# Nuralamsiddik16/Ultrafnd_git

Hardware: AMD Instinct MI355X
Metric: train-step samples/sec (FakeSV batch, seq128+224^2) (higher is better)
Workload: dtype bf16

## Files before the change

### ultrafnd_git_amd/csrc/attn_softmax.hpp

```cpp
#pragma once
#include "common.hpp"

#pragma clang fp contract(off)

__device__ __forceinline__ bf16x8 lds_frag(const char* tile, int row, int chunk) {
  return *reinterpret_cast<const bf16x8*>(tile + row * 128 + ((chunk ^ ((row >> 1) & 7)) << 4));
}

__device__ __forceinline__ bool masked_block_is_noop(const float* kb, int lane, const float (&m_run)[2]) {
  return __all(kb[lane] != 0.0f) && __all(m_run[0] > -1.0e30f && m_run[1] > -1.0e30f);
}

template <int KT, bool DROP = false, bool CAUSAL = false>
__device__ __forceinline__ float online_softmax_block(f32x4 (&s)[KT][2], const int qt, const float* kbias, const bool any_masked, const int g,
                                                      const float scale_log2e, float& m_run, float& l_run, bf16x8 (&pf)[KT / 2][2],
                                                      const f32x4* dm = nullptr, const int qk = 0, const float causal_neg = 0.0f) {
  float mx = -INFINITY, lsum = 0.0f, m_new, alpha;
  if (any_masked) {
#pragma unroll
    for (int kt = 0; kt < KT; ++kt) {
      const f32x4 kbv = *reinterpret_cast<const f32x4*>(kbias + kt * 16 + 4 * g);
#pragma unroll
      for (int r = 0; r < 4; ++r) {
        float v = (kbv[r] == 0.0f) ? s[kt][qt][r] * scale_log2e : kbv[r];
        if constexpr (CAUSAL) {
          if (kbv[r] == 0.0f && 16 * kt + r > qk) v = causal_neg;
        }
        s[kt][qt][r] = v;
        mx = fmaxf(mx, v);
      }
    }
    mx = fmaxf(mx, __shfl_xor(mx, 16, 64));
    mx = fmaxf(mx, __shfl_xor(mx, 32, 64));
    m_new = fmaxf(m_run, mx);
    alpha = fast_exp2(m_run - m_new);
#pragma unroll
    for (int kt = 0; kt < KT; ++kt)
#pragma unroll
      for (int r = 0; r < 4; ++r) {
        const float p = fast_exp2(s[kt][qt][r] - m_new);
        lsum += p;
        if constexpr (DROP) pf[kt >> 1][qt][(kt & 1) * 4 + r] = (__bf16)(p * dm[kt][r]);
        else pf[kt >> 1][qt][(kt & 1) * 4 + r] = (__bf16)p;
      }
  } else {
#pragma unroll
    for (int kt = 0; kt < KT; ++kt)
#pragma unroll
      for (int r = 0; r < 4; ++r) mx = fmaxf(mx, s[kt][qt][r]);
    mx = fmaxf(mx, __shfl_xor(mx, 16, 64));
    mx = fmaxf(mx, __shfl_xor(mx, 32, 64));
    m_new = fmaxf(m_run, mx * scale_log2e);
    alpha = fast_exp2(m_run - m_new);
    const float neg_m = -m_new;
#pragma unroll
    for (int kt = 0; kt < KT; ++kt)
#pragma unroll
      for (int r = 0; r < 4; ++r) {
        const float p = fast_exp2(__builtin_fmaf(s[kt][qt][r], scale_log2e, neg_m));
        lsum += p;
        if constexpr (DROP) pf[kt >> 1][qt][(kt & 1) * 4 + r] = (__bf16)(p * dm[kt][r]);
        else pf[kt >> 1][qt][(kt & 1) * 4 + r] = (__bf16)p;
      }
  }
  l_run = __builtin_fmaf(l_run, alpha, lsum);
  m_run = m_new;
  return alpha;
}

__device__ __forceinline__ void attn_init(f32x4 (&o)[4][2], float (&m_run)[2], float (&l_run)[2]) {
#pragma unroll
  for (int dt = 0; dt < 4; ++dt)
#pragma unroll
    for (int qt = 0; qt < 2; ++qt) o[dt][qt] = f32x4{0.f, 0.f, 0.f, 0.f};
#pragma unroll
  for (int qt = 0; qt < 2; ++qt) m_run[qt] = -INFINITY, l_run[qt] = 0.f;
}

template <class QRow>
__device__ __forceinline__ void attn_q_frags(const char* qimg, QRow q_row, int fr, int g, bf16x8 (&qf)[2][2]) {
#pragma unroll
  for (int qt = 0; qt < 2; ++qt) {
    const int row = q_row(qt * 16 + fr);
    qf[qt][0] = lds_frag(qimg, row, g);
    qf[qt][1] = lds_frag(qimg, row, g + 4);
  }
}

template <int KT, class KeyRow>
__device__ __forceinline__ void attn_scores(const char* kimg, KeyRow key_row, const bf16x8 (&qf)[2][2], int fr, int g, f32x4 (&s)[KT][2]) {
#pragma unroll
  for (int kt = 0; kt < KT; ++kt)
#pragma unroll
    for (int qt = 0; qt < 2; ++qt) s[kt][qt] = f32x4{0.f, 0.f, 0.f, 0.f};
#pragma unroll
  for (int kk = 0; kk < 2; ++kk)
#pragma unroll
    for (int kt = 0; kt < KT; ++kt) {
      const bf16x8 kf = lds_frag(kimg, key_row(kt * 16 + fr), g + 4 * kk);
#pragma unroll
      for (int qt = 0; qt < 2; ++qt) s[kt][qt] = __builtin_amdgcn_mfma_f32_16x16x32_bf16(kf, qf[qt][kk], s[kt][qt], 0, 0, 0);
    }
}

template <int KT, bool DROP = false, bool CAUSAL = false>
__device__ __forceinline__ void attn_softmax_rescale(f32x4 (&s)[KT][2], const int qt, const float* kbias, const bool any_masked, const int g,
                                                     const float scale_log2e, float (&m_run)[2], float (&l_run)[2], bf16x8 (&pf)[KT / 2][2],
                                                     f32x4 (&o)[4][2], const f32x4* dm = nullptr, const int qk = 0, const float causal_neg = 0.0f) {
  const float alpha = online_softmax_block<KT, DROP, CAUSAL>(s, qt, kbias, any_masked, g, scale_log2e, m_run[qt], l_run[qt], pf, dm, qk, causal_neg);
  if (!__all(alpha == 1.0f)) {
#pragma unroll
    for (int dt = 0; dt < 4; ++dt) o[dt][qt] *= alpha;
  }
}

template <int KT, class KeyRow>
__device__ __forceinline__ void attn_pv(const char* vimg, KeyRow key_row, const bf16x8 (&pf)[KT / 2][2], f32x4 (&o)[4][2], int fr, int g) {
#pragma unroll
  for (int ksd = 0; ksd < KT / 2; ++ksd) {
#pragma unroll
    for (int dt = 0; dt < 4; ++dt) {
      const int qq = fr >> 2, pp = fr & 3;
      const int k0 = 32 * ksd + 4 * g + qq;
      const int key0 = key_row(k0), key1 = key_row(k0 + 16);
      const int ch = 2 * dt + (pp >> 1);
      const int off0 = key0 * 128 + ((ch ^ (((key0 >> 1) & 3) << 1)) << 4) + 8 * (pp & 1);
      const int off1 = key1 * 128 + ((ch ^ (((key1 >> 1) & 3) << 1)) << 4) + 8 * (pp & 1);
      const s16x4 t0 = __builtin_amdgcn_ds_read_tr16_b64_v4i16((s16x4 __attribute__((address_space(3)))*)(vimg + off0));
      const s16x4 t1 = __builtin_amdgcn_ds_read_tr16_b64_v4i16((s16x4 __attribute__((address_space(3)))*)(vimg + off1));
      union { s16x4 s2[2]; bf16x8 v; } u;
      u.s2[0] = t0;
      u.s2[1] = t1;
#pragma unroll
      for (int qt = 0; qt < 2; ++qt) o[dt][qt] = __builtin_amdgcn_mfma_f32_16x16x32_bf16(u.v, pf[ksd][qt], o[dt][qt], 0, 0, 0);
    }
  }
}

__device__ __forceinline__ float attn_finish(const float l_run, float& l) {
  l = l_run;
  l += __shfl_xor(l, 16, 64);
  l += __shfl_xor(l, 32, 64);
  return 1.0f / l;
}
__device__ __forceinline__ float attn_finish(const float l_run) {
  float l;
  return attn_finish(l_run, l);
}

__device__ __forceinline__ void attn_store_ctx(__bf16* dst, const f32x4 (&o)[4][2], const int qt, const float inv) {
#pragma unroll
  for (int dt = 0; dt < 4; ++dt) {
    bf16x4 ov = {(__bf16)(o[dt][qt][0] * inv), (__bf16)(o[dt][qt][1] * inv), (__bf16)(o[dt][qt][2] * inv), (__bf16)(o[dt][qt][3] * inv)};
    *reinterpret_cast<bf16x4*>(dst + dt * 16) = ov;
  }
}
```

### ultrafnd_git_amd/csrc/common.hpp

```cpp
#pragma once
#include <hip/hip_runtime.h>
#include <stdint.h>
#include <stdio.h>

#include "../../include/ultrafnd_hip.h"

typedef float f32x16 __attribute__((ext_vector_type(16)));
typedef float f32x4 __attribute__((ext_vector_type(4)));
typedef float f32x2 __attribute__((ext_vector_type(2)));
typedef __bf16 bf16x8 __attribute__((ext_vector_type(8)));
typedef __bf16 bf16x4 __attribute__((ext_vector_type(4)));
typedef short s16x4 __attribute__((ext_vector_type(4)));

#define UFND_WAVE 64

void ufnd_set_error(const char* fmt, ...);
#define UFND_REQUIRE(cond, ...)                      \
  do {                                               \
    if (!(cond)) {                                   \
      ufnd_set_error(__VA_ARGS__);                   \
      return UFND_ERR_INVALID;                       \
    }                                                \
  } while (0)
#define UFND_CHECK_LAUNCH()                                              \
// ... 2 lines not shown
    if (e_ != hipSuccess) {                                              \
      ufnd_set_error("%s:%d launch failed: %s", __FILE__, __LINE__,      \
                     hipGetErrorString(e_));                             \
      return UFND_ERR_LAUNCH;                                            \
    }                                                                    \
  } while (0)

static inline bool ufnd_aligned(const void* p, size_t a) { return (reinterpret_cast<uintptr_t>(p) % a) == 0; }
static inline int ufnd_cdiv(int a, int b) { return (a + b - 1) / b; }

__device__ __forceinline__ float gelu_f(float x) {
  return 0.5f * x * (1.0f + erff(x * 0.70710678118654752440f));
}
__device__ __forceinline__ float gelu_grad_f(float x) {
  const float cdf = 0.5f * (1.0f + erff(x * 0.70710678118654752440f));
  const float pdf = 0.39894228040143267794f * __expf(-0.5f * x * x);
  return cdf + x * pdf;
}
__device__ __forceinline__ float sigmoid_f(float x) { return 1.0f / (1.0f + __expf(-x)); }
__device__ __forceinline__ int xcd_contiguous_id(int n, int total) {
  const int q = total >> 3, r = total & 7, xcd = n & 7, idx = n >> 3;
  return (xcd < r ? xcd * (q + 1) : r * (q + 1) + (xcd - r) * q) + idx;
}

__device__ __forceinline__ float fast_exp2(float x) { return __builtin_amdgcn_exp2f(x); }
__device__ __forceinline__ float quick_gelu_grad_f(float x) {
  const float s = 1.0f / (1.0f + __expf(-1.702f * x));
  return s * (1.0f + 1.702f * x * (1.0f - s));
}
__device__ __forceinline__ float sigmoid_fast_f(float x) {
#pragma clang fp contract(off)
  return __builtin_amdgcn_rcpf(__fadd_rn(1.0f, __expf(-x)));
}
__device__ __forceinline__ float quick_gelu_fast_f(float x) {
#pragma clang fp contract(off)
  return __fmul_rn(x, sigmoid_fast_f(__fmul_rn(1.702f, x)));
}
__device__ __forceinline__ float gelu_fast_f(float x) {
#pragma clang fp contract(off)
  const float z = __fmul_rn(fabsf(x), 0.70710678118654752440f);
  const float t = __builtin_amdgcn_rcpf(__fmaf_rn(0.3275911f, z, 1.0f));
  float p = __fmaf_rn(t, 1.061405429f, -1.453152027f);
  p = __fmaf_rn(t, p, 1.421413741f);
  p = __fmaf_rn(t, p, -0.284496736f);
  p = __fmaf_rn(t, p, 0.254829592f);
  const float poly = __fmul_rn(t, p);
  const float erf_abs = __fmaf_rn(-poly, __expf(__fmul_rn(-z, z)), 1.0f);
  const float h = __fmul_rn(0.5f, x);
  return __fmaf_rn(h, copysignf(erf_abs, x), h);
}

__device__ __forceinline__ f32x2 gelu_fast_f2(f32x2 x) {
#pragma clang fp contract(off)
  const f32x2 z = __builtin_elementwise_abs(x) * 0.70710678118654752440f;
  const f32x2 u = __builtin_elementwise_fma(f32x2{0.3275911f, 0.3275911f}, z, f32x2{1.0f, 1.0f});
  const f32x2 t = {__builtin_amdgcn_rcpf(u.x), __builtin_amdgcn_rcpf(u.y)};
  f32x2 p = __builtin_elementwise_fma(t, f32x2{1.061405429f, 1.061405429f}, f32x2{-1.453152027f, -1.453152027f});
  p = __builtin_elementwise_fma(t, p, f32x2{1.421413741f, 1.421413741f});
  p = __builtin_elementwise_fma(t, p, f32x2{-0.284496736f, -0.284496736f});
  p = __builtin_elementwise_fma(t, p, f32x2{0.254829592f, 0.254829592f});
  const f32x2 poly = t * p;
  const f32x2 zz = (-z) * z;
  const f32x2 e = {__expf(zz.x), __expf(zz.y)};
  const f32x2 erf_abs = __builtin_elementwise_fma(-poly, e, f32x2{1.0f, 1.0f});
  const f32x2 h = x * 0.5f;
  const f32x2 sg = {copysignf(erf_abs.x, x.x), copysignf(erf_abs.y, x.y)};
  return __builtin_elementwise_fma(h, sg, h);
}
__device__ __forceinline__ f32x2 quick_gelu_fast_f2(f32x2 x) {
#pragma clang fp contract(off)
  const f32x2 m = x * 1.702f;
  const f32x2 d = f32x2{__expf(-m.x), __expf(-m.y)} + 1.0f;
  const f32x2 r = {__builtin_amdgcn_rcpf(d.x), __builtin_amdgcn_rcpf(d.y)};
  return x * r;
}

__device__ __forceinline__ float quad_xor1(float v) {
  return __builtin_bit_cast(float, __builtin_amdgcn_update_dpp(0, __builtin_bit_cast(int, v), 0xB1, 0xF, 0xF, false));
}
__device__ __forceinline__ float quad_xor2(float v) {
  return __builtin_bit_cast(float, __builtin_amdgcn_update_dpp(0, __builtin_bit_cast(int, v), 0x4E, 0xF, 0xF, false));
}

#define UFND_DPP(v, old, ctrl, rmask) \
  __builtin_bit_cast(float, __builtin_amdgcn_update_dpp(__builtin_bit_cast(int, (float)(old)), __builtin_bit_cast(int, (float)(v)), ctrl, rmask, 0xF, false))
__device__ __forceinline__ float wave_sum(float v) {
  v += UFND_DPP(v, 0.0f, 0xB1, 0xF);
  v += UFND_DPP(v, 0.0f, 0x4E, 0xF);
  v += UFND_DPP(v, 0.0f, 0x141, 0xF);
  v += UFND_DPP(v, 0.0f, 0x140, 0xF);
  v += UFND_DPP(v, 0.0f, 0x142, 0xA);
  v += UFND_DPP(v, 0.0f, 0x143, 0xC);
  return __builtin_bit_cast(float, __builtin_amdgcn_readlane(__builtin_bit_cast(int, v), 63));
}
__device__ __forceinline__ float wave_max(float v) {
  v = fmaxf(v, UFND_DPP(v, v, 0xB1, 0xF));
  v = fmaxf(v, UFND_DPP(v, v, 0x4E, 0xF));
  v = fmaxf(v, UFND_DPP(v, v, 0x141, 0xF));
  v = fmaxf(v, UFND_DPP(v, v, 0x140, 0xF));
  v = fmaxf(v, UFND_DPP(v, v, 0x142, 0xA));
  v = fmaxf(v, UFND_DPP(v, v, 0x143, 0xC));
  return __builtin_bit_cast(float, __builtin_amdgcn_readlane(__builtin_bit_cast(int, v), 63));
}

__device__ __forceinline__ void philox_4x32(uint64_t seed, uint64_t step, uint32_t layer, uint32_t ctr, uint32_t (&out)[4]) {
  uint32_t k0 = (uint32_t)seed, k1 = (uint32_t)(seed >> 32);
  uint32_t c0 = ctr, c1 = layer, c2 = (uint32_t)step, c3 = (uint32_t)(step >> 32);
#pragma unroll
  for (int r = 0; r < 10; ++r) {
    const uint64_t p0 = (uint64_t)0xD2511F53u * c0;
    const uint64_t p1 = (uint64_t)0xCD9E8D57u * c2;
    const uint32_t n0 = (uint32_t)(p1 >> 32) ^ c1 ^ k0;
    const uint32_t n1 = (uint32_t)p1;
    const uint32_t n2 = (uint32_t)(p0 >> 32) ^ c3 ^ k1;
    const uint32_t n3 = (uint32_t)p0;
    c0 = n0; c1 = n1; c2 = n2; c3 = n3;
    k0 += 0x9E3779B9u; k1 += 0xBB67AE85u;
  }
  out[0] = c0; out[1] = c1; out[2] = c2; out[3] = c3;
}
__device__ __forceinline__ float dropout_keep(uint32_t r, float p) {
  const float u = (float)(r >> 8) * (1.0f / 16777216.0f);
  return (u >= p) ? 1.0f / (1.0f - p) : 0.0f;
}
__device__ __forceinline__ uint64_t dropout_step_key(const ufnd_step_state* st) { return st->step + ((uint64_t)st->micro << 40); }
__device__ __forceinline__ float dropout_mul(const ufnd_step_state* st, float p, uint32_t layer, uint32_t elem) {
  if (p <= 0.0f) return 1.0f;
  uint32_t w[4];
  philox_4x32(st->seed, dropout_step_key(st), layer, elem >> 2, w);
  const uint32_t k = elem & 3u;
  return dropout_keep(k == 0 ? w[0] : (k == 1 ? w[1] : (k == 2 ? w[2] : w[3])), p);
}
__device__ __forceinline__ void dropout_mul4(const ufnd_step_state* st, float p, uint32_t layer, uint32_t elem4, float (&m)[4]) {
  if (p <= 0.0f) { m[0] = m[1] = m[2] = m[3] = 1.0f; return; }
  uint32_t w[4];
  philox_4x32(st->seed, dropout_step_key(st), layer, elem4 >> 2, w);
#pragma unroll
  for (int q = 0; q < 4; ++q) m[q] = dropout_keep(w[q], p);
}
__device__ __forceinline__ void dropout_mul4_ctr(uint64_t seed, uint64_t step, float p, uint32_t layer, uint32_t ctr, float (&m)[4]) {
  uint32_t w[4];
  philox_4x32(seed, step, layer, ctr, w);
#pragma unroll
  for (int q = 0; q < 4; ++q) m[q] = dropout_keep(w[q], p);
}

static inline bool ufnd_attn_dropout_fits(int B, int L, int heads) {
  const long long lp = (L + 3) / 4 * 4;
  return (long long)B * heads * L * lp / 4 <= (1ll << 32);
}
constexpr uint32_t UFND_TAG_TEXT = 256;
constexpr uint32_t UFND_TAG_VISION = 4096;
```

### ultrafnd_git_amd/csrc/diag/gemm_diag.hip

```cpp
#define UFND_DIAG 1
#include "../gemm_bf16_kernel.hpp"
#include "../gemm_bf16_checks.hpp"

extern "C" int ufnd_diag_gemm_bf16_ex(const void* A, const void* W, const float* bias, const float* residual, void* out_bf16,
                                      float* out_f32, int M, int N, int K, int lda, int ldw, int ldr, int ldo, int ldf, int act,
                                      int tile_cfg, void* stream_) {
  UFND_REQUIRE(A && W && (out_bf16 || out_f32), "diag gemm: null operand");
  UFND_REQUIRE(M >= 1 && N >= 64 && K >= 64 && N % 64 == 0 && K % 64 == 0, "diag gemm: M=%d N=%d K=%d", M, N, K);
  GemmArgs a{(const __bf16*)A, (const __bf16*)W, bias, residual, (__bf16*)out_bf16, out_f32, M, N, K, lda, ldw, ldr, ldo, ldf, act, 0, 0, nullptr};
  int mode = 0, cfg = tile_cfg < 0 ? auto_cfg(M, N, K) : tile_cfg;
  if (cfg >= 200) { mode = 2; cfg -= 200; } else if (cfg >= 100) { mode = 1; cfg -= 100; }
  UFND_REQUIRE(cfg < kNumTiles, "diag gemm: unknown tile config %d", cfg);
  UFND_REQUIRE(N % kTiles[cfg].bn == 0, "diag gemm: tile config %d needs N %% %d == 0", cfg, kTiles[cfg].bn);
  int rc = launch_cfg(cfg, mode, a, (hipStream_t)stream_);
  if (rc != UFND_OK) return rc;
  UFND_CHECK_LAUNCH();
  return UFND_OK;
}

extern "C" int ufnd_diag_gemm_bf16_stamps(const void* A, const void* W, void* out_bf16, int M, int N, int K, int tile_cfg,
                                     unsigned long long* stamps, const ufnd_gemm_ln* ln, const float* bias, const float* residual,
                                     float* out_f32, void* stream_) {
  UFND_REQUIRE(A && W && out_bf16 && stamps, "gemm_bf16_stamps: null operand");
  UFND_REQUIRE(M >= 1 && N >= 64 && K >= 64 && N % 64 == 0 && K % 64 == 0, "gemm_bf16_stamps: M=%d N=%d K=%d", M, N, K);
  UFND_REQUIRE(tile_cfg >= 0 && tile_cfg < kNumTiles && N % kTiles[tile_cfg].bn == 0, "gemm_bf16_stamps: tile config %d", tile_cfg);
  GemmArgs a{(const __bf16*)A, (const __bf16*)W, bias, residual, (__bf16*)out_bf16, out_f32, M, N, K, K, K, N, N, N, 0, 0, 0, stamps};
  int abl = 3;
  if (ln) {
    UFND_REQUIRE(kTiles[tile_cfg].lnx, "gemm_bf16_stamps: tile %d has no LayerNorm-aware kernel", tile_cfg);
    a.a_stats = ln->a_stats; a.colsum = ln->colsum; a.r_stats = ln->r_stats; a.r_gamma = ln->r_gamma; a.r_beta = ln->r_beta;
    a.out_stats = ln->out_stats; a.a_parts = ln->a_parts; a.r_parts = ln->r_parts; a.a_eps = ln->a_eps; a.r_eps = ln->r_eps;
    a.inv_h = 1.0f / (float)ln->width;
    a.residual_b = (const __bf16*)ln->residual_bf16;
    a.ldrb = ln->ldrb;
    a.guard = ln->a_stats ? ln->guard : nullptr;
    if (ln->tile_cfg > 0) a.act = ln->tile_cfg;
    abl = 5;
  }
  int rc = launch_cfg(tile_cfg, abl, a, (hipStream_t)stream_);
  if (rc != UFND_OK) return rc;
  UFND_CHECK_LAUNCH();
  return UFND_OK;
}

extern "C" int ufnd_diag_qkv_attention_stamps(const void* X, const void* Wqkv, const float* bqkv, const int32_t* key_mask, void* ctx, int B,
                                              int heads, const ufnd_gemm_ln* ln, unsigned long long* stamps, void* stream_) {
  UFND_REQUIRE(X && Wqkv && ctx && stamps && heads % 2 == 0, "diag qkv_attention: bad argument");
  const int H = heads * 64;
  GemmArgs a{(const __bf16*)X, (const __bf16*)Wqkv, bqkv, nullptr, nullptr, nullptr, B * 128, 3 * H, H, H, H, 0, 0, 0, UFND_ACT_NONE, 0, 0, stamps};
  if (ln && ln->a_stats) {
    a.a_stats = ln->a_stats; a.colsum = ln->colsum; a.a_parts = ln->a_parts; a.a_eps = ln->a_eps;
    a.inv_h = 1.0f / (float)ln->width;
    a.guard = ln->guard;
  }
  a.att_mask = key_mask;
  a.att_ctx = (__bf16*)ctx;
  a.att_h = H;
  a.att_scale_log2e = 0.125f * 1.44269504088896340736f;
  a.m_tiles = B;
  a.n_tiles = heads / 2;
  a.xcd_cols = (a.n_tiles % 2 == 0 && a.m_tiles >= 4) ? 2 : 1;
  hipLaunchKernelGGL((gemm_bf16_kernel<128, 384, 2, 4, 3, 2, 16, 0, 1, 1, 1>), dim3(a.m_tiles * a.n_tiles), dim3(512), 0, (hipStream_t)stream_, a);
  UFND_CHECK_LAUNCH();
  return UFND_OK;
}

extern "C" int ufnd_diag_qkv_attention_tiles_stamps(const void* X, const void* Wqkv, const float* bqkv, const int32_t* tiles, const int32_t* ntiles,
                                                    void* ctx, int cap_tiles, int heads, const ufnd_gemm_ln* ln, unsigned long long* stamps,
                                                    void* stream_) {
  UFND_REQUIRE(X && Wqkv && ctx && stamps && tiles && ntiles && cap_tiles >= 1 && heads >= 1, "diag qkv_attention_tiles: bad argument");
  const int H = heads * 64;
  GemmArgs a{(const __bf16*)X, (const __bf16*)Wqkv, bqkv, nullptr, nullptr, nullptr, cap_tiles * 256, 3 * H, H, H, H, 0, 0, 0, UFND_ACT_NONE, 0, 0, stamps};
  if (ln && ln->a_stats) {
    a.a_stats = ln->a_stats; a.colsum = ln->colsum; a.a_parts = ln->a_parts; a.a_eps = ln->a_eps;
    a.inv_h = 1.0f / (float)ln->width;
    a.guard = ln->guard;
  }
  a.att_bins = tiles;
  a.att_nbins = ntiles;
  a.att_ctx = (__bf16*)ctx;
  a.att_h = H;
  a.att_scale_log2e = 0.125f * 1.44269504088896340736f;
  a.m_tiles = cap_tiles;
  a.n_tiles = heads;
  a.xcd_cols = 1;
  hipLaunchKernelGGL((gemm_bf16_kernel<256, 192, 4, 2, 3, 2, 16, 0, 1, 1, 2>), dim3(a.m_tiles * a.n_tiles), dim3(512), 0, (hipStream_t)stream_, a);
  UFND_CHECK_LAUNCH();
  return UFND_OK;
}

int ufnd_diag_pp_shape_ok(int M, int N, int K);
extern "C" int ufnd_diag_gemm_bf16_plan(int entry, const void* A, const void* W, const float* bias, const float* residual, const void* aux,
                                        const void* out_bf16, const float* out_f32, int M, int N, int K, int lda, int ldw, int ldr, int ldaux,
                                        int ldo, int ldf, int act, int tile_cfg, const ufnd_gemm_ln* ln, int* out) {
  UFND_REQUIRE(out, "gemm_bf16_plan: null result pointer");
  UFND_REQUIRE(entry >= -1 && entry <= 3, "gemm_bf16_plan: entry %d", entry);
  int cfg = tile_cfg, rc = UFND_OK, parts = 0;
  if (entry == -1) {
    UFND_REQUIRE(cfg >= 0 && cfg < kNumTiles, "gemm_bf16_plan: no tile %d", cfg);
    M = N = K = 0;
  } else if (entry == 3) {
    rc = gemm_bf16_dgrad_check_args(A, W, residual, aux, out_bf16, out_f32, M, N, K, lda, ldw, ldr, ldaux, ldo, ldf, act);
    if (rc != UFND_OK) return rc;
    cfg = auto_cfg(M, N, K);
    rc = gemm_bf16_dgrad_check_tile(cfg, N);
    if (rc != UFND_OK) return rc;
  } else {
    if (entry == 2) {
      rc = gemm_bf16_ln_check_args(A, W, bias, residual, out_bf16, out_f32, M, N, K, lda, ldw, ldr, ldo, ldf, act, ln);
      if (rc != UFND_OK) return rc;
      cfg = ln->tile_cfg;
    } else {
      rc = gemm_bf16_check_args(A, W, bias, residual, out_bf16, out_f32, M, N, K, lda, ldw, ldr, ldo, ldf, act);
      if (rc != UFND_OK) return rc;
      if (entry == 0) cfg = -1;
    }
    UFND_REQUIRE(cfg != UFND_GEMM_TILE_PERSISTENT && !(cfg < 0 && ufnd_diag_pp_shape_ok(M, N, K)),
                 "gemm_bf16_plan: the persistent form may take this call (its choice needs the device): not planned here");
    if (cfg < 0) cfg = auto_cfg(M, N, K);
    rc = entry == 2 ? gemm_bf16_ln_check_tile(cfg, M, N, K, ln) : gemm_bf16_check_tile(cfg, N);
    if (rc != UFND_OK) return rc;
    if (entry == 2 && ln->out_stats) parts = stat_parts_for(cfg, N);
  }
  const TileCfg& t = kTiles[cfg];
  const int m_tiles = entry < 0 ? 0 : ufnd_cdiv(M, t.bm), n_tiles = entry < 0 ? 0 : N / t.bn;
  out[0] = cfg;
  out[1] = m_tiles;
  out[2] = n_tiles;
  out[3] = entry < 0 ? 0 : xcd_cols_for(M, N, K, m_tiles, n_tiles);
  out[4] = parts;
  out[5] = t.bm; out[6] = t.bn; out[7] = t.sta; out[8] = t.stb; out[9] = t.lnx; out[10] = t.prod; out[11] = gemm_bwd_tile(cfg) ? 1 : 0;
  return UFND_OK;
}
```

### ultrafnd_git_amd/csrc/gemm_bf16_kernel.hpp

```cpp
#pragma once
#ifndef UFND_GEMM_OUT_NT
#define UFND_GEMM_OUT_NT 0
#endif

#include <type_traits>

#include "common.hpp"
#include "attn_softmax.hpp"

#pragma clang fp contract(off)

#ifndef UFND_GEMM_ILV
#define UFND_GEMM_ILV 1
#endif

namespace {

constexpr int BK = 64;

struct GemmArgs {
  const __bf16* A;
  const __bf16* W;
  const float* bias;
  const float* residual;
// ... 186 lines not shown
    }
    return tr < alen;
  };
  const int wave = __builtin_amdgcn_readfirstlane(threadIdx.x >> 6), lane = threadIdx.x & 63;
  const int wm = wave / WN, wn = wave % WN, fr = lane & (MI - 1), g = lane / MI;

  acc_t acc[MT][NT];
#pragma unroll
  for (int i = 0; i < MT; ++i)
#pragma unroll
    for (int j = 0; j < NT; ++j)
#pragma unroll
      for (int r = 0; r < AR; ++r) acc[i][j][r] = 0.f;

  int nk = a.K / BK, kbase = 0;
  if constexpr (BWD) {
    if (a.ksplit > 1) {
      const int per = (nk + a.ksplit - 1) / a.ksplit;
      kbase = kslice * per * BK;
      nk = nk - kslice * per < per ? nk - kslice * per : per;
    }
  }
  const int prow = lane >> 3, ppos = lane & 7;
  int arow_att[ATT ? PWA : 1];
  if constexpr (ATT) {
#pragma unroll
    for (int ii = 0; ii < PWA; ++ii) arow_att[ii] = tile_row(8 * (wave + NW * ii) + prow);
  }
  auto issueA = [&](int t, int kt) {
    char* buf = smem + (t % STA) * ASLOT;
    const int k0 = kbase + kt * BK;
#pragma unroll
    for (int ii = 0; ii < PWA; ++ii) {
      const int p = wave + NW * ii;
      const int r = 8 * p + prow;
      const int c = ppos ^ ((r >> 1) & 7);
      int gr = arow0 + r;
      gr = gr < mlive ? gr : mlive - 1;
      if constexpr (ATT) gr = arow_att[ii];
      dma16(a.A + (size_t)gr * a.lda + k0 + c * 8, buf + p * 1024);
    }
  };
  auto issueB = [&](int t, int kt) {
    char* buf = smem + STA * ASLOT + (t % STB) * BSLOT;
    const int k0 = kbase + kt * BK;
#pragma unroll
    for (int ii = 0; ii < PWB; ++ii) {
      int p = wave + NW * ii;
      if constexpr (BPIECES % NW != 0) p = p < BPIECES ? p : p - BPIECES;
      const int r = 8 * p + prow;
      const int c = ppos ^ ((r >> 1) & 7);
      int gr = n0 + r;
      gr = gr < a.N ? gr : a.N - 1;
      if constexpr (ONEH) gr = (r >> 6) * a.att_h + tn * 64 + (r & 63);
      else if constexpr (ATT) gr = (r >> 7) * a.att_h + tn * 128 + (r & 127);
      dma16(a.W + (size_t)gr * a.ldw + k0 + c * 8, buf + p * 1024);
    }
  };
  constexpr int TPR = NW * 64 / BM;
  static_assert(!LNX || TPR == 2 || TPR == 4, "threads per tile row");
  constexpr int GPT = 4 / (TPR < 4 ? TPR : 4);
  f32x4 sv[GPT][3];
  f32x2* st_lds = reinterpret_cast<f32x2*>(smem + STAT_OFF);
  const float* sp = nullptr;
  if constexpr (LNX) {
    sp = a.a_stats ? a.a_stats : a.r_stats;
    if (sp) {
      const int parts = a.a_stats ? a.a_parts : a.r_parts;
      int row = arow0 + (int)threadIdx.x / TPR;
      row = row < mlive ? row : mlive - 1;
      if constexpr (ATT) row = tile_row((int)threadIdx.x / TPR);
      const f32x4* base = reinterpret_cast<const f32x4*>(sp + (size_t)row * parts * 2);
      const int nq = parts >> 1, sub = threadIdx.x % TPR;
#pragma unroll
      for (int gi = 0; gi < GPT; ++gi)
#pragma unroll
        for (int u = 0; u < 3; ++u) {
          const int q = (sub + gi * TPR) + 4 * u;
          asm volatile("global_load_dwordx4 %0, %1, off" : "=v"(sv[gi][u]) : "v"(base + (q < nq ? q : 0)) : "memory");
        }
    }
  }
  float til_kb = 0.0f;
  if constexpr (TIL) {
    if (threadIdx.x < BM) til_kb = __int_as_float(til[UFND_TEXT_TILE_KBIAS + threadIdx.x]);
  }
  int att_mk = 1;
  if constexpr (ATT == 1 && !VIT) {
    if (slots) {
      const int j = (int)threadIdx.x >> 7, k = threadIdx.x & 127;
      const int mt = j == 0 ? smeta[0] : j == 1 ? smeta[1] : j == 2 ? smeta[2] : smeta[3];
      att_mk = mt >= 0 && k < (mt & 255);
      if (att_mk && a.att_mask) att_mk = a.att_mask[(size_t)(mt >> 10) * BM + k];
    } else if (a.att_mask && threadIdx.x < BM) {
      att_mk = a.att_mask[m0 + threadIdx.x];
    }
  }
#pragma unroll
  for (int s = 0; s < STA; ++s) {
    const int ks = s < nk ? s : nk - 1;
    if (s < STB && (LNX || s < nk)) issueB(s, ks);
    if (LNX || s < nk) issueA(s, ks);
  }

  if constexpr (LNX) {
    if (sp) {
      constexpr int NPRO = STA * PWA + STB * PWB;
      static_assert(NPRO <= 63, "vmcnt range");
      if constexpr (GPT == 1)
        asm volatile("s_waitcnt vmcnt(%3) ; STATRETIRE %0 %1 %2" : "+v"(sv[0][0]), "+v"(sv[0][1]), "+v"(sv[0][2]) : "n"(NPRO) : "memory");
      else
        asm volatile("s_waitcnt vmcnt(%6) ; STATRETIRE %0 %1 %2 %3 %4 %5" : "+v"(sv[0][0]), "+v"(sv[0][1]), "+v"(sv[0][2]), "+v"(sv[GPT - 1][0]),
                     "+v"(sv[GPT - 1][1]), "+v"(sv[GPT - 1][2]) : "n"(NPRO) : "memory");
      const int nq_ = (a.a_stats ? a.a_parts : a.r_parts) >> 1, sub_ = threadIdx.x % TPR;
      float gs[GPT], gq[GPT];
#pragma unroll
      for (int gi = 0; gi < GPT; ++gi) {
#pragma unroll
        for (int u = 0; u < 3; ++u) {
          if ((sub_ + gi * TPR) + 4 * u >= nq_) sv[gi][u] = f32x4{0.f, 0.f, 0.f, 0.f};
        }
        gs[gi] = sv[gi][0][0] + sv[gi][0][2];
        gq[gi] = sv[gi][0][1] + sv[gi][0][3];
#pragma unroll
        for (int u = 1; u < 3; ++u) { gs[gi] += sv[gi][u][0] + sv[gi][u][2]; gq[gi] += sv[gi][u][1] + sv[gi][u][3]; }
      }
      float sm, sq;
      if constexpr (TPR == 4) {
        sm = gs[0] + quad_xor1(gs[0]);
        sq = gq[0] + quad_xor1(gq[0]);
        sm += quad_xor2(sm);
        sq += quad_xor2(sq);
      } else {
        const float s01 = gs[0] + quad_xor1(gs[0]), s23 = gs[1] + quad_xor1(gs[1]);
        const float q01 = gq[0] + quad_xor1(gq[0]), q23 = gq[1] + quad_xor1(gq[1]);
        sm = s01 + s23;
        sq = q01 + q23;
      }
      const float mean = __fmul_rn(sm, a.inv_h);
      const float var = fmaxf(__fmaf_rn(-mean, mean, __fmul_rn(sq, a.inv_h)), 0.f);
      const float rstd = __builtin_amdgcn_rsqf(__fadd_rn(var, a.a_stats ? a.a_eps : a.r_eps));
      if (threadIdx.x % TPR == 0) st_lds[threadIdx.x / TPR] = f32x2{mean, rstd};
      if (a.guard && a.a_stats) {
        float ratio = __fmul_rn(fabsf(mean), rstd);
        ratio = ratio == ratio ? ratio : INFINITY;
        const float worst = wave_max(threadIdx.x % TPR == 0 && tile_row_live((int)threadIdx.x / TPR) ? ratio : 0.0f);
        if (lane == 0) reinterpret_cast<float*>(smem + STAT_OFF + BM * 8)[wave] = worst;
      }
      asm volatile("s_waitcnt lgkmcnt(0)" ::: "memory");
    }
  }

  bf16x8 af0[KQ][MT], bf0[KQ][NT], af1[KQ][MT], bf1[KQ][NT];
  auto read_half = [&](int t, auto kk_, bf16x8 (&af)[KQ][MT], bf16x8 (&bfr)[KQ][NT]) {
    constexpr int kk = decltype(kk_)::value;
    const char* At = smem + (t % STA) * ASLOT;
    const char* Bt = smem + STA * ASLOT + (t % STB) * BSLOT;
#pragma unroll
    for (int q = 0; q < KQ; ++q) {
      const int chunk = MI == 16 ? g + 4 * kk : g + 2 * q + 4 * kk;
#pragma unroll
      for (int i = 0; i < MT; ++i) af[q][i] = lds_frag(At, wm * TM + i * MI + fr, chunk);
#pragma unroll
      for (int j = 0; j < NT; ++j) bfr[q][j] = lds_frag(Bt, wn * TN + j * MI + fr, chunk);
    }
  };
  auto mma_half = [&](const bf16x8 (&af)[KQ][MT], const bf16x8 (&bfr)[KQ][NT]) {
#pragma unroll
// ... 223 lines not shown
        if constexpr (RES) if ((a.residual && !(BWD && a.aux)) || (LNX && a.residual_b)) {
          if constexpr (RLN) {
            const f32x2 ms = st_lds[wm * TM + i * MI + rr];
            if constexpr (!FIXCOL) {
              ld8(a.r_gamma + col, g8);
              ld8(a.r_beta + col, b8);
            }
#pragma unroll
            for (int q = 0; q < 8; ++q) rr8[it][q] = __fmaf_rn(__fmul_rn(__fsub_rn(rr8[it][q], ms[0]), ms[1]), g8[q], b8[q]);
          }
#pragma unroll
          for (int q = 0; q < 8; ++q) v[q] = __fadd_rn(v[q], rr8[it][q]);
        }
        if constexpr (LNX && RES) {
          if (a.out_stats) {
            if constexpr (CPR % 4 == 0) {
              float sm = 0.f, sq = 0.f;
#pragma unroll
              for (int q = 0; q < 8; ++q) { sm = __fadd_rn(sm, v[q]); sq = __fmaf_rn(v[q], v[q], sq); }
              sm += quad_xor1(sm);
              sq += quad_xor1(sq);
              sm += quad_xor2(sm);
              sq += quad_xor2(sq);
              if (live && (id & 3) == 0)
                *reinterpret_cast<f32x2*>(a.out_stats + ((size_t)row * (a.N >> 5) + (col >> 5)) * 2) = f32x2{sm, sq};
            }
          }
        }
        if constexpr (ATT) {
          const int ct = wn * TN + cl;
          const int trow = wm * TM + i * MI + rr, img = ct >> 6, ch = (ct & 63) >> 3;
          bf16x8 o;
#pragma unroll
          for (int q = 0; q < 8; ++q) o[q] = (__bf16)v[q];
          const int sw = img >= (ONEH ? 2 : 4) ? (ch ^ (((trow >> 1) & 3) << 1)) : (ch ^ ((trow >> 1) & 7));
          *reinterpret_cast<bf16x8*>(smem + ATT_OFF + img * ATT_IMG + trow * 128 + (sw << 4)) = o;
          continue;
        }
        if (!live) continue;
        if (a.out_f32) {
          float* op = outf + (size_t)row * a.ldf + col;
          *reinterpret_cast<f32x4*>(op) = f32x4{v[0], v[1], v[2], v[3]};
          *reinterpret_cast<f32x4*>(op + 4) = f32x4{v[4], v[5], v[6], v[7]};
        }
        if (a.out_bf16) {
          bf16x8 o;
#pragma unroll
          for (int q = 0; q < 8; ++q) o[q] = (__bf16)v[q];
          if constexpr (UFND_GEMM_OUT_NT && !BWD) __builtin_nontemporal_store(o, reinterpret_cast<bf16x8*>(a.out_bf16 + (size_t)row * a.ldo + col));
          else *reinterpret_cast<bf16x8*>(a.out_bf16 + (size_t)row * a.ldo + col) = o;
        }
      }
      asm volatile("s_waitcnt lgkmcnt(0)" ::: "memory");
    }
  };
  if constexpr (LNX) {
    if (fold) {
      if (a.act == UFND_ACT_GELU) epilogue(IntC<UFND_ACT_GELU>{}, IntC<1>{});
      else if (a.act == UFND_ACT_QUICK_GELU) epilogue(IntC<UFND_ACT_QUICK_GELU>{}, IntC<1>{});
      else epilogue(IntC<UFND_ACT_NONE>{}, IntC<1>{});
    } else if (rln) {
      epilogue(IntC<UFND_ACT_NONE>{}, IntC<2>{});
    } else {
      epilogue(IntC<UFND_ACT_NONE>{}, IntC<0>{});
    }
  } else {
    if (a.act == UFND_ACT_GELU) epilogue(IntC<UFND_ACT_GELU>{}, IntC<0>{});
    else if (a.act == UFND_ACT_QUICK_GELU) epilogue(IntC<UFND_ACT_QUICK_GELU>{}, IntC<0>{});
    else epilogue(IntC<UFND_ACT_NONE>{}, IntC<0>{});
  }
  if constexpr (ATT && DBG) {
    stamp[8] = __builtin_amdgcn_s_memtime();
    stamp[9] = __builtin_amdgcn_s_memrealtime();
  }
  if constexpr (VIT) {
    const int T = a.att_t;
    float* kbias = reinterpret_cast<float*>(smem + ATT_OFF + 3 * ATT_IMG);
    if (threadIdx.x < 64) kbias[threadIdx.x] = (int)threadIdx.x < T ? 0.0f : -INFINITY;
    __syncthreads();
    const int g4 = lane >> 4, f16 = lane & 15;
    const char* qimg = smem + ATT_OFF;
    const char* kimg = smem + ATT_OFF + ATT_IMG;
    const char* vimg = smem + ATT_OFF + 2 * ATT_IMG;
    const int nqb = (T + 31) >> 5, nsamp = alen > 0 ? alen / T : 0;
    const bool any_masked = __any(kbias[lane] != 0.0f);
    constexpr int KT = 4;
    for (int u = wave; u < nsamp * nqb; u += NW) {
      const int smp = u / nqb, q0 = (u - smp * nqb) * 32, r0 = smp * T;
      const auto row = [&](int k) { return r0 + (k < T ? k : T - 1); };
      bf16x8 qf[2][2];
      attn_q_frags(qimg, [&](int q) { return row(q0 + q); }, f16, g4, qf);
      f32x4 o[4][2], sc[KT][2];
      float m_run[2], l_run[2];
      bf16x8 pf[KT / 2][2];
      attn_init(o, m_run, l_run);
      attn_scores<KT>(kimg, row, qf, f16, g4, sc);
#pragma unroll
      for (int qt = 0; qt < 2; ++qt) attn_softmax_rescale<KT>(sc, qt, kbias, any_masked, g4, a.att_scale_log2e, m_run, l_run, pf, o);
      attn_pv<KT>(vimg, row, pf, o, f16, g4);
#pragma unroll
      for (int qt = 0; qt < 2; ++qt) {
        const float inv = attn_finish(l_run[qt]);
        const int q = q0 + qt * 16 + f16;
        if (q < T) attn_store_ctx(a.att_ctx + (size_t)(arow0 + r0 + q) * a.att_h + tn * 64 + 4 * g4, o, qt, inv);
      }
    }
  } else if constexpr (TIL) {
    constexpr float NEG_MASK = -3.0e38f;
    float* kbias = reinterpret_cast<float*>(smem + ATT_OFF + 3 * ATT_IMG);
    float* wbias = kbias + BM + wave * 128;
    if (threadIdx.x < BM) kbias[threadIdx.x] = til_kb;
    __syncthreads();
    const int g4 = lane >> 4, f16 = lane & 15;
    const char* qimg = smem + ATT_OFF;
    const char* kimg = smem + ATT_OFF + ATT_IMG;
    const char* vimg = smem + ATT_OFF + 2 * ATT_IMG;
    int nunits = __builtin_amdgcn_readfirstlane(til[2]);
    nunits = nunits < UFND_TEXT_TILE_UNITS ? nunits : UFND_TEXT_TILE_UNITS;
    constexpr int KB = 64, KT = KB / 16;
    for (int u = wave; u < nunits; u += NW) {
      const int unit = __builtin_amdgcn_readfirstlane(til[UFND_TEXT_TILE_UNIT0 + u]);
      const int sj = unit & (UFND_TEXT_TILE_SAMPLES - 1), q0 = ((unit >> 8) & 3) * 32;
      const int grow0 = __builtin_amdgcn_readfirstlane(til[4 + 2 * sj]);
      const int meta = __builtin_amdgcn_readfirstlane(til[5 + 2 * sj]);
      const int r0 = (meta >> 8) & 255;
      int n = meta & 255;
      n = n < 1 ? 1 : (n < BM - r0 ? n : BM - r0);
      n = n < 128 ? n : 128;
#pragma unroll
      for (int h = 0; h < 2; ++h) {
        const int k = lane + 64 * h;
        wbias[k] = k < n ? kbias[r0 + k] : NEG_MASK;
      }
      asm volatile("s_waitcnt lgkmcnt(0)" ::: "memory");
      const auto row = [&](int k) { return r0 + (k < n ? k : n - 1); };
      bf16x8 qf[2][2];
      attn_q_frags(qimg, [&](int q) { return row(q0 + q); }, f16, g4, qf);
      f32x4 o[4][2];
      float m_run[2], l_run[2];
      attn_init(o, m_run, l_run);
#pragma unroll
      for (int kb0 = 0; kb0 < 128; kb0 += KB) {
        if (masked_block_is_noop(wbias + kb0, lane, m_run)) continue;
        const auto key_row = [&](int k) { return row(kb0 + k); };
        f32x4 sc[KT][2];
        attn_scores<KT>(kimg, key_row, qf, f16, g4, sc);
        const bool any_masked = __any(wbias[kb0 + lane] != 0.0f);
        bf16x8 pf[KT / 2][2];
#pragma unroll
        for (int qt = 0; qt < 2; ++qt) attn_softmax_rescale<KT>(sc, qt, wbias + kb0, any_masked, g4, a.att_scale_log2e, m_run, l_run, pf, o);
        attn_pv<KT>(vimg, key_row, pf, o, f16, g4);
      }
#pragma unroll
      for (int qt = 0; qt < 2; ++qt) {
        const float inv = attn_finish(l_run[qt]);
        const int q = q0 + qt * 16 + f16;
        if (q < n) attn_store_ctx(a.att_ctx + (size_t)(grow0 + q) * a.att_h + tn * 64 + 4 * g4, o, qt, inv);
      }
    }
  } else if constexpr (ATT) {
    constexpr float NEG_MASK = -3.0e38f;
    float* kbias = reinterpret_cast<float*>(smem + ATT_OFF + 6 * 16384);
    if (slots || threadIdx.x < BM) kbias[threadIdx.x] = att_mk != 0 ? 0.0f : NEG_MASK;
    __syncthreads();
    const int hh = wave >> 2, wq = wave & 3, g4 = lane >> 4, f16 = lane & 15;
    int wrow0 = arow0 + 32 * wq, wcnt = alen - 32 * wq, koff = 0;
    const float* wbias = kbias;
    if (slots) {
      const int mt = wq == 0 ? smeta[0] : wq == 1 ? smeta[1] : wq == 2 ? smeta[2] : smeta[3];
      wrow0 = wq == 0 ? srow[0] : wq == 1 ? srow[1] : wq == 2 ? srow[2] : srow[3];
      wcnt = wq == 0 ? scnt[0] : wq == 1 ? scnt[1] : wq == 2 ? scnt[2] : scnt[3];
      koff = 32 * (wq - ((mt >> 8) & 3));
      wbias = kbias + wq * BM;
    }
    const char* qimg = smem + ATT_OFF + hh * 16384;
    const char* kimg = smem + ATT_OFF + (2 + hh) * 16384;
    const char* vimg = smem + ATT_OFF + (4 + hh) * 16384;
    bf16x8 qf[2][2];
    attn_q_frags(qimg, [&](int q) { return wq * 32 + q; }, f16, g4, qf);
    f32x4 o[4][2];
    float m_run[2], l_run[2];
    attn_init(o, m_run, l_run);
    constexpr int KB = 64, KT = KB / 16;
    if (wcnt > 0) {
#pragma unroll
      for (int kb0 = 0; kb0 < BM; kb0 += KB) {
        if (masked_block_is_noop(wbias + kb0, lane, m_run)) continue;
        const int kr0 = koff + kb0;
        const auto key_row = [&](int k) { return (kr0 + k) & (BM - 1); };
        f32x4 sc[KT][2];
        attn_scores<KT>(kimg, key_row, qf, f16, g4, sc);
        const bool any_masked = __any(wbias[kb0 + lane] != 0.0f);
        bf16x8 pf[KT / 2][2];
#pragma unroll
        for (int qt = 0; qt < 2; ++qt) attn_softmax_rescale<KT>(sc, qt, wbias + kb0, any_masked, g4, a.att_scale_log2e, m_run, l_run, pf, o);
        attn_pv<KT>(vimg, key_row, pf, o, f16, g4);
      }
    }
#pragma unroll
    for (int qt = 0; qt < 2; ++qt) {
      const float inv = attn_finish(l_run[qt]);
      const int q = qt * 16 + f16;
      if (q < wcnt) attn_store_ctx(a.att_ctx + (size_t)(wrow0 + q) * a.att_h + (tn * 2 + hh) * 64 + 4 * g4, o, qt, inv);
    }
  }
  if constexpr (LNX) {
    if (a.guard && a.a_stats && threadIdx.x == 0) {
// ... 163 lines not shown
```

Baseline: 30840.

## Split ViT attention into 16-query units, use permlane swaps and lane-held tile metadata

The ViT fused QKV-attention path now assigns one 16-query tile per wave unit instead of two, so the short 50-token sequences give more units, waste fewer padded query rows, and balance better across waves. The attention helpers are templated on the number of query tiles to allow this. Cross-lane max and sum reductions switch from __shfl_xor to permlane16/32 swap builtins, avoiding LDS-based shuffles. Text-tile metadata is loaded once into one word per lane and read with readlane instead of repeated scalar global loads. The smaller units re-read K and V fragments more often per query, and a diagnostic timing entry point is added.

```diff
diff --git a/ultrafnd_git_amd/csrc/attn_softmax.hpp b/ultrafnd_git_amd/csrc/attn_softmax.hpp
--- a/ultrafnd_git_amd/csrc/attn_softmax.hpp
+++ b/ultrafnd_git_amd/csrc/attn_softmax.hpp
@@ -7,13 +7,16 @@
   return *reinterpret_cast<const bf16x8*>(tile + row * 128 + ((chunk ^ ((row >> 1) & 7)) << 4));
 }
 
-__device__ __forceinline__ bool masked_block_is_noop(const float* kb, int lane, const float (&m_run)[2]) {
-  return __all(kb[lane] != 0.0f) && __all(m_run[0] > -1.0e30f && m_run[1] > -1.0e30f);
+template <int NQT = 2>
+__device__ __forceinline__ bool masked_block_is_noop(const float* kb, int lane, const float (&m_run)[NQT]) {
+  bool seen = m_run[0] > -1.0e30f;
+  if constexpr (NQT == 2) seen = seen && m_run[1] > -1.0e30f;
+  return __all(kb[lane] != 0.0f) && __all(seen);
 }
 
-template <int KT, bool DROP = false, bool CAUSAL = false>
-__device__ __forceinline__ float online_softmax_block(f32x4 (&s)[KT][2], const int qt, const float* kbias, const bool any_masked, const int g,
-                                                      const float scale_log2e, float& m_run, float& l_run, bf16x8 (&pf)[KT / 2][2],
+template <int KT, bool DROP = false, bool CAUSAL = false, int NQT = 2>
+__device__ __forceinline__ float online_softmax_block(f32x4 (&s)[KT][NQT], const int qt, const float* kbias, const bool any_masked, const int g,
+                                                      const float scale_log2e, float& m_run, float& l_run, bf16x8 (&pf)[KT / 2][NQT],
                                                       const f32x4* dm = nullptr, const int qk = 0, const float causal_neg = 0.0f) {
   float mx = -INFINITY, lsum = 0.0f, m_new, alpha;
   if (any_masked) {
@@ -30,8 +33,8 @@
         mx = fmaxf(mx, v);
       }
     }
-    mx = fmaxf(mx, __shfl_xor(mx, 16, 64));
-    mx = fmaxf(mx, __shfl_xor(mx, 32, 64));
+    mx = fmaxf(mx, lane_xor16(mx));
+    mx = fmaxf(mx, lane_xor32(mx));
     m_new = fmaxf(m_run, mx);
     alpha = fast_exp2(m_run - m_new);
 #pragma unroll
@@ -48,8 +51,8 @@
     for (int kt = 0; kt < KT; ++kt)
 #pragma unroll
       for (int r = 0; r < 4; ++r) mx = fmaxf(mx, s[kt][qt][r]);
-    mx = fmaxf(mx, __shfl_xor(mx, 16, 64));
-    mx = fmaxf(mx, __shfl_xor(mx, 32, 64));
+    mx = fmaxf(mx, lane_xor16(mx));
+    mx = fmaxf(mx, lane_xor32(mx));
     m_new = fmaxf(m_run, mx * scale_log2e);
     alpha = fast_exp2(m_run - m_new);
     const float neg_m = -m_new;
@@ -68,54 +71,55 @@
   return alpha;
 }
 
-__device__ __forceinline__ void attn_init(f32x4 (&o)[4][2], float (&m_run)[2], float (&l_run)[2]) {
+template <int NQT = 2>
+__device__ __forceinline__ void attn_init(f32x4 (&o)[4][NQT], float (&m_run)[NQT], float (&l_run)[NQT]) {
 #pragma unroll
   for (int dt = 0; dt < 4; ++dt)
 #pragma unroll
-    for (int qt = 0; qt < 2; ++qt) o[dt][qt] = f32x4{0.f, 0.f, 0.f, 0.f};
+    for (int qt = 0; qt < NQT; ++qt) o[dt][qt] = f32x4{0.f, 0.f, 0.f, 0.f};
 #pragma unroll
-  for (int qt = 0; qt < 2; ++qt) m_run[qt] = -INFINITY, l_run[qt] = 0.f;
+  for (int qt = 0; qt < NQT; ++qt) m_run[qt] = -INFINITY, l_run[qt] = 0.f;
 }
 
-template <class QRow>
-__device__ __forceinline__ void attn_q_frags(const char* qimg, QRow q_row, int fr, int g, bf16x8 (&qf)[2][2]) {
+template <class QRow, int NQT = 2>
+__device__ __forceinline__ void attn_q_frags(const char* qimg, QRow q_row, int fr, int g, bf16x8 (&qf)[NQT][2]) {
 #pragma unroll
-  for (int qt = 0; qt < 2; ++qt) {
+  for (int qt = 0; qt < NQT; ++qt) {
     const int row = q_row(qt * 16 + fr);
     qf[qt][0] = lds_frag(qimg, row, g);
     qf[qt][1] = lds_frag(qimg, row, g + 4);
   }
 }
 
-template <int KT, class KeyRow>
-__device__ __forceinline__ void attn_scores(const char* kimg, KeyRow key_row, const bf16x8 (&qf)[2][2], int fr, int g, f32x4 (&s)[KT][2]) {
+template <int KT, class KeyRow, int NQT = 2>
+__device__ __forceinline__ void attn_scores(const char* kimg, KeyRow key_row, const bf16x8 (&qf)[NQT][2], int fr, int g, f32x4 (&s)[KT][NQT]) {
 #pragma unroll
   for (int kt = 0; kt < KT; ++kt)
 #pragma unroll
-    for (int qt = 0; qt < 2; ++qt) s[kt][qt] = f32x4{0.f, 0.f, 0.f, 0.f};
+    for (int qt = 0; qt < NQT; ++qt) s[kt][qt] = f32x4{0.f, 0.f, 0.f, 0.f};
 #pragma unroll
   for (int kk = 0; kk < 2; ++kk)
 #pragma unroll
     for (int kt = 0; kt < KT; ++kt) {
       const bf16x8 kf = lds_frag(kimg, key_row(kt * 16 + fr), g + 4 * kk);
 #pragma unroll
-      for (int qt = 0; qt < 2; ++qt) s[kt][qt] = __builtin_amdgcn_mfma_f32_16x16x32_bf16(kf, qf[qt][kk], s[kt][qt], 0, 0, 0);
+      for (int qt = 0; qt < NQT; ++qt) s[kt][qt] = __builtin_amdgcn_mfma_f32_16x16x32_bf16(kf, qf[qt][kk], s[kt][qt], 0, 0, 0);
     }
 }
 
-template <int KT, bool DROP = false, bool CAUSAL = false>
-__device__ __forceinline__ void attn_softmax_rescale(f32x4 (&s)[KT][2], const int qt, const float* kbias, const bool any_masked, const int g,
-                                                     const float scale_log2e, float (&m_run)[2], float (&l_run)[2], bf16x8 (&pf)[KT / 2][2],
-                                                     f32x4 (&o)[4][2], const f32x4* dm = nullptr, const int qk = 0, const float causal_neg = 0.0f) {
-  const float alpha = online_softmax_block<KT, DROP, CAUSAL>(s, qt, kbias, any_masked, g, scale_log2e, m_run[qt], l_run[qt], pf, dm, qk, causal_neg);
+template <int KT, bool DROP = false, bool CAUSAL = false, int NQT = 2>
+__device__ __forceinline__ void attn_softmax_rescale(f32x4 (&s)[KT][NQT], const int qt, const float* kbias, const bool any_masked, const int g,
+                                                     const float scale_log2e, float (&m_run)[NQT], float (&l_run)[NQT], bf16x8 (&pf)[KT / 2][NQT],
+                                                     f32x4 (&o)[4][NQT], const f32x4* dm = nullptr, const int qk = 0, const float causal_neg = 0.0f) {
+  const float alpha = online_softmax_block<KT, DROP, CAUSAL, NQT>(s, qt, kbias, any_masked, g, scale_log2e, m_run[qt], l_run[qt], pf, dm, qk, causal_neg);
   if (!__all(alpha == 1.0f)) {
 #pragma unroll
     for (int dt = 0; dt < 4; ++dt) o[dt][qt] *= alpha;
   }
 }
 
-template <int KT, class KeyRow>
-__device__ __forceinline__ void attn_pv(const char* vimg, KeyRow key_row, const bf16x8 (&pf)[KT / 2][2], f32x4 (&o)[4][2], int fr, int g) {
+template <int KT, int NQT = 2, class KeyRow>
+__device__ __forceinline__ void attn_pv(const char* vimg, KeyRow key_row, const bf16x8 (&pf)[KT / 2][NQT], f32x4 (&o)[4][NQT], int fr, int g) {
 #pragma unroll
   for (int ksd = 0; ksd < KT / 2; ++ksd) {
 #pragma unroll
@@ -132,15 +136,15 @@
       u.s2[0] = t0;
       u.s2[1] = t1;
 #pragma unroll
-      for (int qt = 0; qt < 2; ++qt) o[dt][qt] = __builtin_amdgcn_mfma_f32_16x16x32_bf16(u.v, pf[ksd][qt], o[dt][qt], 0, 0, 0);
+      for (int qt = 0; qt < NQT; ++qt) o[dt][qt] = __builtin_amdgcn_mfma_f32_16x16x32_bf16(u.v, pf[ksd][qt], o[dt][qt], 0, 0, 0);
     }
   }
 }
 
 __device__ __forceinline__ float attn_finish(const float l_run, float& l) {
   l = l_run;
-  l += __shfl_xor(l, 16, 64);
-  l += __shfl_xor(l, 32, 64);
+  l += lane_xor16(l);
+  l += lane_xor32(l);
   return 1.0f / l;
 }
 __device__ __forceinline__ float attn_finish(const float l_run) {
@@ -148,7 +152,8 @@
   return attn_finish(l_run, l);
 }
 
-__device__ __forceinline__ void attn_store_ctx(__bf16* dst, const f32x4 (&o)[4][2], const int qt, const float inv) {
+template <int NQT = 2>
+__device__ __forceinline__ void attn_store_ctx(__bf16* dst, const f32x4 (&o)[4][NQT], const int qt, const float inv) {
 #pragma unroll
   for (int dt = 0; dt < 4; ++dt) {
     bf16x4 ov = {(__bf16)(o[dt][qt][0] * inv), (__bf16)(o[dt][qt][1] * inv), (__bf16)(o[dt][qt][2] * inv), (__bf16)(o[dt][qt][3] * inv)};
diff --git a/ultrafnd_git_amd/csrc/common.hpp b/ultrafnd_git_amd/csrc/common.hpp
--- a/ultrafnd_git_amd/csrc/common.hpp
+++ b/ultrafnd_git_amd/csrc/common.hpp
@@ -108,6 +108,17 @@
   return __builtin_bit_cast(float, __builtin_amdgcn_update_dpp(0, __builtin_bit_cast(int, v), 0x4E, 0xF, 0xF, false));
 }
 
+__device__ __forceinline__ float lane_xor16(float v) {
+  const unsigned x = __builtin_bit_cast(unsigned, v);
+  const auto r = __builtin_amdgcn_permlane16_swap(x, x, false, false);
+  return __builtin_bit_cast(float, (__lane_id() & 16) ? r[0] : r[1]);
+}
+__device__ __forceinline__ float lane_xor32(float v) {
+  const unsigned x = __builtin_bit_cast(unsigned, v);
+  const auto r = __builtin_amdgcn_permlane32_swap(x, x, false, false);
+  return __builtin_bit_cast(float, (__lane_id() & 32) ? r[0] : r[1]);
+}
+
 #define UFND_DPP(v, old, ctrl, rmask) \
   __builtin_bit_cast(float, __builtin_amdgcn_update_dpp(__builtin_bit_cast(int, (float)(old)), __builtin_bit_cast(int, (float)(v)), ctrl, rmask, 0xF, false))
 __device__ __forceinline__ float wave_sum(float v) {
diff --git a/ultrafnd_git_amd/csrc/diag/gemm_diag.hip b/ultrafnd_git_amd/csrc/diag/gemm_diag.hip
--- a/ultrafnd_git_amd/csrc/diag/gemm_diag.hip
+++ b/ultrafnd_git_amd/csrc/diag/gemm_diag.hip
@@ -89,6 +89,28 @@
   return UFND_OK;
 }
 
+extern "C" int ufnd_diag_qkv_attention_vit_stamps(const void* X, const void* Wqkv, const float* bqkv, void* ctx, int N, int T, int heads,
+                                                  const ufnd_gemm_ln* ln, unsigned long long* stamps, void* stream_) {
+  UFND_REQUIRE(X && Wqkv && ctx && stamps && N >= 1 && T >= 1 && T <= 64 && heads >= 1, "diag qkv_attention_vit: bad argument");
+  const int H = heads * 64;
+  GemmArgs a{(const __bf16*)X, (const __bf16*)Wqkv, bqkv, nullptr, nullptr, nullptr, N * T, 3 * H, H, H, H, 0, 0, 0, UFND_ACT_NONE, 0, 0, stamps};
+  if (ln && ln->a_stats) {
+    a.a_stats = ln->a_stats; a.colsum = ln->colsum; a.a_parts = ln->a_parts; a.a_eps = ln->a_eps;
+    a.inv_h = 1.0f / (float)ln->width;
+    a.guard = ln->guard;
+  }
+  a.att_ctx = (__bf16*)ctx;
+  a.att_h = H;
+  a.att_scale_log2e = 0.125f * 1.44269504088896340736f;
+  a.att_t = T;
+  a.m_tiles = ufnd_cdiv(N, 256 / T);
+  a.n_tiles = heads;
+  a.xcd_cols = 1;
+  hipLaunchKernelGGL((gemm_bf16_kernel<256, 192, 4, 2, 3, 2, 16, 0, 1, 1, 1>), dim3(a.m_tiles * a.n_tiles), dim3(512), 0, (hipStream_t)stream_, a);
+  UFND_CHECK_LAUNCH();
+  return UFND_OK;
+}
+
 int ufnd_diag_pp_shape_ok(int M, int N, int K);
 extern "C" int ufnd_diag_gemm_bf16_plan(int entry, const void* A, const void* W, const float* bias, const float* residual, const void* aux,
                                         const void* out_bf16, const float* out_f32, int M, int N, int K, int lda, int ldw, int ldr, int ldaux,
diff --git a/ultrafnd_git_amd/csrc/gemm_bf16_kernel.hpp b/ultrafnd_git_amd/csrc/gemm_bf16_kernel.hpp
--- a/ultrafnd_git_amd/csrc/gemm_bf16_kernel.hpp
+++ b/ultrafnd_git_amd/csrc/gemm_bf16_kernel.hpp
@@ -292,8 +292,11 @@
     }
   }
   float til_kb = 0.0f;
+  int til_w = 0;
   if constexpr (TIL) {
+    static_assert(UFND_TEXT_TILE_UNIT0 + UFND_TEXT_TILE_UNITS <= 64 && 4 + 2 * UFND_TEXT_TILE_SAMPLES <= UFND_TEXT_TILE_UNIT0, "one word per lane");
     if (threadIdx.x < BM) til_kb = __int_as_float(til[UFND_TEXT_TILE_KBIAS + threadIdx.x]);
+    til_w = til[lane];
   }
   int att_mk = 1;
   if constexpr (ATT == 1 && !VIT) {
@@ -683,24 +686,25 @@
     const char* qimg = smem + ATT_OFF;
     const char* kimg = smem + ATT_OFF + ATT_IMG;
     const char* vimg = smem + ATT_OFF + 2 * ATT_IMG;
-    const int nqb = (T + 31) >> 5, nsamp = alen > 0 ? alen / T : 0;
+    constexpr int NQT = 1, UQ = 16 * NQT;
+    const int nqb = (T + UQ - 1) / UQ, nsamp = alen > 0 ? alen / T : 0;
     const bool any_masked = __any(kbias[lane] != 0.0f);
     constexpr int KT = 4;
     for (int u = wave; u < nsamp * nqb; u += NW) {
-      const int smp = u / nqb, q0 = (u - smp * nqb) * 32, r0 = smp * T;
+      const int smp = u / nqb, q0 = (u - smp * nqb) * UQ, r0 = smp * T;
       const auto row = [&](int k) { return r0 + (k < T ? k : T - 1); };
-      bf16x8 qf[2][2];
+      bf16x8 qf[NQT][2];
       attn_q_frags(qimg, [&](int q) { return row(q0 + q); }, f16, g4, qf);
-      f32x4 o[4][2], sc[KT][2];
-      float m_run[2], l_run[2];
-      bf16x8 pf[KT / 2][2];
+      f32x4 o[4][NQT], sc[KT][NQT];
+      float m_run[NQT], l_run[NQT];
+      bf16x8 pf[KT / 2][NQT];
       attn_init(o, m_run, l_run);
       attn_scores<KT>(kimg, row, qf, f16, g4, sc);
 #pragma unroll
-      for (int qt = 0; qt < 2; ++qt) attn_softmax_rescale<KT>(sc, qt, kbias, any_masked, g4, a.att_scale_log2e, m_run, l_run, pf, o);
+      for (int qt = 0; qt < NQT; ++qt) attn_softmax_rescale<KT>(sc, qt, kbias, any_masked, g4, a.att_scale_log2e, m_run, l_run, pf, o);
       attn_pv<KT>(vimg, row, pf, o, f16, g4);
 #pragma unroll
-      for (int qt = 0; qt < 2; ++qt) {
+      for (int qt = 0; qt < NQT; ++qt) {
         const float inv = attn_finish(l_run[qt]);
         const int q = q0 + qt * 16 + f16;
         if (q < T) attn_store_ctx(a.att_ctx + (size_t)(arow0 + r0 + q) * a.att_h + tn * 64 + 4 * g4, o, qt, inv);
@@ -716,14 +720,14 @@
     const char* qimg = smem + ATT_OFF;
     const char* kimg = smem + ATT_OFF + ATT_IMG;
     const char* vimg = smem + ATT_OFF + 2 * ATT_IMG;
-    int nunits = __builtin_amdgcn_readfirstlane(til[2]);
-    nunits = nunits < UFND_TEXT_TILE_UNITS ? nunits : UFND_TEXT_TILE_UNITS;
+    int nunits = __builtin_amdgcn_readlane(til_w, 2);
+    nunits = nunits < 0 ? 0 : (nunits < UFND_TEXT_TILE_UNITS ? nunits : UFND_TEXT_TILE_UNITS);
     constexpr int KB = 64, KT = KB / 16;
     for (int u = wave; u < nunits; u += NW) {
-      const int unit = __builtin_amdgcn_readfirstlane(til[UFND_TEXT_TILE_UNIT0 + u]);
+      const int unit = __builtin_amdgcn_readlane(til_w, UFND_TEXT_TILE_UNIT0 + u);
       const int sj = unit & (UFND_TEXT_TILE_SAMPLES - 1), q0 = ((unit >> 8) & 3) * 32;
-      const int grow0 = __builtin_amdgcn_readfirstlane(til[4 + 2 * sj]);
-      const int meta = __builtin_amdgcn_readfirstlane(til[5 + 2 * sj]);
+      const int grow0 = __builtin_amdgcn_readlane(til_w, 4 + 2 * sj);
+      const int meta = __builtin_amdgcn_readlane(til_w, 5 + 2 * sj);
       const int r0 = (meta >> 8) & 255;
       int n = meta & 255;
       n = n < 1 ? 1 : (n < BM - r0 ? n : BM - r0);
```

Result: no change. 31070 (median of 6 runs) (+0.7%).
